# pyg-team/pytorch_geometric

Hardware: NVIDIA H100
Metric: edges/sec (GCNConv fwd+bwd) (higher is better)
Workload: dtype f32

## Files before the change

include/b200mp.h:

```cpp
#ifndef B200MP_H_
#define B200MP_H_

#include <stdint.h>

#ifdef __cplusplus
extern "C" {
#endif

#define B200MP_VERSION "0.1.0"

enum { B200MP_F32 = 0, B200MP_BF16 = 1 };
enum { B200MP_I32 = 0, B200MP_I64 = 1 };
enum { B200MP_SUM = 0, B200MP_MEAN = 1, B200MP_MIN = 2, B200MP_MAX = 3, B200MP_MUL = 4 };
enum {
    B200MP_OK = 0,
    B200MP_ERR_INVALID_ARG = -1,
    B200MP_ERR_UNSUPPORTED = -2,
    B200MP_ERR_CUDA = -3,
    B200MP_ERR_WORKSPACE = -4
};

const char* b200mp_version(void);
const char* b200mp_last_error(void);
int b200mp_device_info(int* sm_count, int* cc_major, int* cc_minor, int64_t* l2_bytes);
// ... 18 lines not shown
                         void* stream);
int64_t b200mp_self_loops_workspace_bytes(int64_t n_edges, int64_t n_nodes, int idx_dtype);
int b200mp_self_loops(const void* row, const void* col, const float* w_in, int64_t n_edges,
                      int64_t n_nodes, float fill_value, int mode, void* row_out, void* col_out,
                      float* w_out, int64_t* n_out_dev, void* workspace, int64_t workspace_bytes,
                      int idx_dtype, void* stream);
int b200mp_gcn_norm_csr(const void* rowptr, const void* src, const float* w, int64_t n_nodes,
                        int64_t n_edges, float* deg_inv_sqrt, float* w_out, int idx_dtype,
                        void* stream);

int b200mp_csr_plan_count(const void* rowptr, int64_t n_rows, int64_t chunk, int64_t* counts_dev,
                          int idx_dtype, void* stream);
int64_t b200mp_csr_plan_workspace_bytes(int64_t n_rows, int64_t n_long_rows, int idx_dtype);
int b200mp_csr_plan_fill(const void* rowptr, int64_t n_rows, int64_t chunk, int64_t n_long_rows,
                         int64_t* long_rows, int64_t* chunk_ptr, void* workspace,
                         int64_t workspace_bytes, int idx_dtype, void* stream);

int b200mp_spmm_csr(const void* rowptr, const void* col, const float* val, const void* x,
                    void* out, int64_t n_rows, int64_t n_cols, int64_t feat, int reduce,
                    const int64_t* long_rows, const int64_t* chunk_ptr, int64_t n_long_rows,
                    int64_t n_chunks, int64_t chunk, float* partials, const float* bias,
                    const void* x_halo, int64_t n_local_cols, int flags, const void* peer_ptrs,
                    int64_t peer_rows, const void* relu_mask, int idx_dtype, int val_dtype, void* stream);

int b200mp_segment_csr(const void* ptr, const void* src, void* out, int64_t n_rows, int64_t n_src,
                       int64_t feat, int reduce, const int64_t* long_rows, const int64_t* chunk_ptr,
                       int64_t n_long_rows, int64_t n_chunks, int64_t chunk, float* partials,
                       int idx_dtype, int val_dtype, void* stream);

int b200mp_minmax_ties(const void* rowptr, const void* col, const float* val, const void* x,
                       const void* out, float* ties, int64_t n_rows, int64_t feat,
                       int count_self_zero, int idx_dtype, int val_dtype, void* stream);
int b200mp_minmax_backward(const void* rowptr_t, const void* col_t, const float* val_t,
                           const void* x, const void* out, const void* grad_out, const float* ties,
                           void* grad_x, int64_t n_src, int64_t feat, int idx_dtype,
                           int val_dtype, void* stream);

int b200mp_sddmm_csr(const void* rowptr, const void* col, const void* a, const void* b, float* dot,
                     int64_t n_rows, int64_t feat, int idx_dtype, int val_dtype, void* stream);

int b200mp_edge_relu_csr(const void* rowptr, const void* col, const void* perm, const void* x,
                         const void* edge_rows, void* out, void* mask, int64_t n_rows, int64_t n_cols,
                         int64_t n_edges, int64_t feat, int reduce, const int64_t* long_rows,
                         const int64_t* chunk_ptr, int64_t n_long_rows, int64_t n_chunks, int64_t chunk,
                         float* partials, int idx_dtype, int val_dtype, void* stream);
int b200mp_edge_relu_backward_x(const void* rowptr_t, const void* col_t, const void* t2csr,
// ... 264 lines not shown
```

pytorch_geometric_b200/_lib.py:

```python
from __future__ import annotations

import ctypes
import os
import re

from . import _build

_I64 = ctypes.c_int64
_INT = ctypes.c_int
_P = ctypes.c_void_p
_F = ctypes.c_float
_U64 = ctypes.c_uint64

_SIGS = {
    "b200mp_version": (ctypes.c_char_p, []),
    "b200mp_last_error": (ctypes.c_char_p, []),
    "b200mp_device_info": (_INT, [_P, _P, _P, _P]),
    "b200mp_set_option": (_INT, [ctypes.c_char_p, _INT]),
    "b200mp_degree": (_INT, [_P, _I64, _I64, _P, _INT, _P]),
    "b200mp_index2ptr": (_INT, [_P, _I64, _I64, _P, _INT, _P]),
    "b200mp_ptr2index": (_INT, [_P, _I64, _I64, _P, _INT, _P]),
    "b200mp_index_stats": (_INT, [_P, _I64, _P, _INT, _P]),
    "b200mp_sort_workspace_bytes": (_I64, [_I64, _I64, _INT]),
    "b200mp_sort_by_key": (_INT, [_P, _I64, _I64, _P, _P, _P, _P, _I64, _INT, _P]),
    "b200mp_permute": (_INT, [_P, _P, _P, _I64, _INT, _INT, _P]),
    "b200mp_convert_index": (_INT, [_P, _INT, _P, _INT, _I64, _P]),
    "b200mp_self_loops_workspace_bytes": (_I64, [_I64, _I64, _INT]),
    "b200mp_self_loops": (_INT, [_P, _P, _P, _I64, _I64, _F, _INT, _P, _P, _P, _P, _P, _I64, _INT, _P]),
    "b200mp_gcn_norm_csr": (_INT, [_P, _P, _P, _I64, _I64, _P, _P, _INT, _P]),
    "b200mp_csr_plan_count": (_INT, [_P, _I64, _I64, _P, _INT, _P]),
    "b200mp_csr_plan_workspace_bytes": (_I64, [_I64, _I64, _INT]),
    "b200mp_csr_plan_fill": (_INT, [_P, _I64, _I64, _I64, _P, _P, _P, _I64, _INT, _P]),
    "b200mp_spmm_csr": (_INT, [_P, _P, _P, _P, _P, _I64, _I64, _I64, _INT, _P, _P, _I64, _I64, _I64, _P,
                               _P, _P, _I64, _INT, _P, _I64, _P, _INT, _INT, _P]),
    "b200mp_segment_csr": (_INT, [_P, _P, _P, _I64, _I64, _I64, _INT, _P, _P, _I64, _I64, _I64, _P, _INT, _INT, _P]),
    "b200mp_minmax_ties": (_INT, [_P, _P, _P, _P, _P, _P, _I64, _I64, _INT, _INT, _INT, _P]),
    "b200mp_minmax_backward": (_INT, [_P, _P, _P, _P, _P, _P, _P, _P, _I64, _I64, _INT, _INT, _P]),
    "b200mp_sddmm_csr": (_INT, [_P, _P, _P, _P, _P, _I64, _I64, _INT, _INT, _P]),
    "b200mp_edge_relu_csr": (_INT, [_P] * 7 + [_I64] * 4 + [_INT, _P, _P, _I64, _I64, _I64, _P, _INT, _INT, _P]),
    "b200mp_edge_relu_backward_x": (_INT, [_P] * 7 + [_I64, _I64, _P, _P, _I64, _I64, _I64, _P, _INT, _INT, _P]),
    "b200mp_edge_relu_backward_edge": (_INT, [_P] * 5 + [_I64, _I64, _INT, _P, _P, _I64, _I64, _I64, _INT, _INT, _P]),
    "b200mp_gated_csr": (_INT, [_P] * 6 + [_I64] * 5 + [_INT, _P, _P, _I64, _I64, _I64, _P, _INT, _INT, _P]),
    "b200mp_gated_backward_dst": (_INT, [_P] * 7 + [_I64] * 5 + [_INT, _P, _P, _I64, _I64, _I64, _P, _INT, _INT, _P]),
    "b200mp_gated_backward_src": (_INT, [_P] * 9 + [_I64] * 5 + [_P, _P, _I64, _I64, _I64, _P, _INT, _INT, _P]),
    "b200mp_cg_csr": (_INT, [_P] * 7 + [_I64] * 6 + [_INT, _P, _P, _I64, _I64, _I64, _P, _INT, _INT, _P]),
    "b200mp_cg_backward_dst": (_INT, [_P] * 9 + [_I64] * 6 + [_INT, _P, _P, _I64, _I64, _I64, _P, _INT, _INT, _P]),
    "b200mp_cg_backward_src": (_INT, [_P] * 9 + [_I64] * 6 + [_P, _P, _I64, _I64, _I64, _P, _INT, _INT, _P]),
    "b200mp_softmax_aggr_csr": (_INT, [_P] * 8 + [_I64] * 4 + [_INT, _F, _INT, _P, _P, _I64, _I64, _I64, _P, _INT, _INT,
                                                                _P]),
    "b200mp_softmax_aggr_workspace": (_I64, [_I64, _I64, _I64]),
    "b200mp_softmax_aggr_backward_dst": (_INT, [_P] * 12 + [_I64] * 4 + [_INT, _F, _INT, _INT, _P, _P, _I64, _I64, _I64,
                                                                           _INT, _INT, _P]),
    "b200mp_softmax_aggr_backward_src": (_INT, [_P] * 10 + [_I64] * 4 + [_INT, _F, _INT, _INT, _P, _P, _I64, _I64, _I64,
                                                                           _P, _INT, _INT, _P]),
    "b200mp_power_mean_csr": (_INT, [_P] * 8 + [_I64] * 4 + [_INT, _F, _INT, _F, _F, _P, _P, _I64, _I64, _I64, _P,
                                                              _INT, _INT, _P]),
    "b200mp_power_mean_workspace": (_I64, [_I64, _I64, _I64, _I64]),
# ... 100 lines not shown
```

pytorch_geometric_b200/csrc/csr_reduce.cuh:

```cuda
#pragma once

#include "common.cuh"

namespace b200mp {

int get_option_spmm_tune();

struct LongRowPlan {
    const int64_t* long_rows;
    const int64_t* chunk_ptr;
    int64_t n_long;
    int64_t n_chunks;
    int64_t chunk;
    float* partials;
    const void* x2;
    int64_t split;
    int accumulate;
    const unsigned long long* peers;
    int64_t peer_rows;
    const void* relu_mask;
};

inline int make_plan(LongRowPlan& plan, const int64_t* long_rows, const int64_t* chunk_ptr, int64_t n_long_rows,
                     int64_t n_chunks, int64_t chunk, float* partials, bool needs_partials) {
// ... 31 lines not shown
        is_chunk = true;
        return true;
    }
    row = item - plan.n_chunks;
    if (row >= n_rows) return false;
    begin = static_cast<int64_t>(__ldg(rowptr + row));
    end = static_cast<int64_t>(__ldg(rowptr + row + 1));
    is_chunk = false;
    if (plan.n_long > 0 && end - begin > plan.chunk) return false;
    return true;
}

template <int RED>
__device__ __forceinline__ float finalize(float acc, int64_t deg, bool is_mean, bool inf_to_zero) {
    if (RED == B200MP_SUM) {
        if (is_mean) acc = __fdiv_rn(acc, static_cast<float>(deg < 1 ? 1 : deg));
    } else if (RED == B200MP_MIN || RED == B200MP_MAX) {
        if (deg == 0) acc = 0.0f;
        if (inf_to_zero && isinf(acc)) acc = 0.0f;
    }
    return acc;
}

template <typename T, typename I, int G, int VPL, int RED, bool GATHER, int UNR_OVR = 0, int BLOCK = 256,
          int MINB = 1>
__global__ void __launch_bounds__(BLOCK, MINB)
csr_reduce_kernel(const I* __restrict__ rowptr, const I* __restrict__ col,
                  const float* __restrict__ val, const T* __restrict__ x, T* __restrict__ out,
                  int64_t n_rows, int n_vec, bool is_mean, bool inf_to_zero, LongRowPlan plan,
                  const float* __restrict__ bias) {
    constexpr int EPV = ElemTraits<T>::kPerVec;
    constexpr int UNR = UNR_OVR ? UNR_OVR : (VPL == 1 ? 8 : (VPL == 2 ? 4 : 2));
    const int lig = threadIdx.x & (G - 1);
    const int64_t item = (static_cast<int64_t>(blockIdx.x) * blockDim.x + threadIdx.x) / G;
    int64_t row, begin, end;
    bool is_chunk;
    const bool active = decode_item(item, rowptr, n_rows, plan, row, begin, end, is_chunk);
    if (G < 32 && !active) return;
    if (G == 32 && !active) return;
    const size_t row_bytes = static_cast<size_t>(n_vec) * 16;
    const char* xb = reinterpret_cast<const char*>(x);
    const char* xb2 = plan.x2 ? reinterpret_cast<const char*>(plan.x2) - static_cast<size_t>(plan.split) * row_bytes : xb;
    const int64_t split = plan.x2 ? plan.split : INT64_MAX;

    for (int vbase = 0; vbase < n_vec; vbase += G * VPL) {
        float acc[VPL][EPV];
#pragma unroll
        for (int k = 0; k < VPL; ++k)
#pragma unroll
            for (int i = 0; i < EPV; ++i) acc[k][i] = red_identity<RED>();
        bool vvalid[VPL];
#pragma unroll
        for (int k = 0; k < VPL; ++k) vvalid[k] = (vbase + lig + k * G) < n_vec;
        const size_t voff = static_cast<size_t>(vbase + lig) * 16;

        if (G == 32) {
            for (int64_t e0 = begin; e0 < end; e0 += 32) {
                const int n = static_cast<int>(end - e0 < 32 ? end - e0 : 32);
                int64_t c_l = 0;
                float w_l = 1.0f;
                if (lig < n) {
                    c_l = GATHER ? static_cast<int64_t>(ldg_idx(col + e0 + lig)) : (e0 + lig);
                    if (val) w_l = __ldg(val + e0 + lig);
                    c_l = static_cast<int64_t>(reinterpret_cast<uintptr_t>(row_base(plan, xb, xb2, split, row_bytes, c_l)));
                }
                for (int j = 0; j < n; j += UNR) {
                    Vec16 buf[UNR][VPL];
                    float w[UNR];
#pragma unroll
                    for (int u = 0; u < UNR; ++u) {
                        const int64_t c = __shfl_sync(0xffffffffu, c_l, (j + u) & 31);
                        w[u] = __shfl_sync(0xffffffffu, w_l, (j + u) & 31);
                        if (j + u < n) {
                            const char* p = reinterpret_cast<const char*>(static_cast<uintptr_t>(c)) + voff;
#pragma unroll
                            for (int k = 0; k < VPL; ++k)
                                if (vvalid[k]) buf[u][k] = ldg_row16(p + static_cast<size_t>(k) * G * 16);
                        }
                    }
#pragma unroll
                    for (int u = 0; u < UNR; ++u) {
                        if (j + u < n) {
#pragma unroll
                            for (int k = 0; k < VPL; ++k) {
                                if (vvalid[k]) {
                                    float f[EPV];
                                    ElemTraits<T>::unpack(buf[u][k], f);
#pragma unroll
                                    for (int i = 0; i < EPV; ++i) {
                                        const float m = val ? __fmul_rn(w[u], f[i]) : f[i];
                                        acc[k][i] = red_combine<RED>(acc[k][i], m);
                                    }
                                }
                            }
                        }
                    }
                }
            }
        } else {
            for (int64_t e = begin; e < end; e += UNR) {
                Vec16 buf[UNR][VPL];
                float w[UNR];
#pragma unroll
                for (int u = 0; u < UNR; ++u) {
                    w[u] = 1.0f;
                    if (e + u < end) {
                        const int64_t c = GATHER ? static_cast<int64_t>(ldg_idx(col + e + u)) : (e + u);
                        if (val) w[u] = __ldg(val + e + u);
                        if (vvalid[0]) buf[u][0] = ldg_row16(row_base(plan, xb, xb2, split, row_bytes, c) + voff);
                    }
                }
#pragma unroll
                for (int u = 0; u < UNR; ++u) {
                    if (e + u < end && vvalid[0]) {
                        float f[EPV];
                        ElemTraits<T>::unpack(buf[u][0], f);
#pragma unroll
                        for (int i = 0; i < EPV; ++i) {
                            const float m = val ? __fmul_rn(w[u], f[i]) : f[i];
                            acc[0][i] = red_combine<RED>(acc[0][i], m);
                        }
                    }
                }
            }
        }

        if (is_chunk) {
            float* pbase = plan.partials + static_cast<size_t>(item) * n_vec * EPV;
#pragma unroll
            for (int k = 0; k < VPL; ++k)
                if (vvalid[k]) store_partial<EPV>(pbase + static_cast<size_t>(vbase + lig + k * G) * EPV, acc[k]);
        } else {
            const int64_t deg = end - begin;
            char* ob = reinterpret_cast<char*>(out) + static_cast<size_t>(row) * row_bytes;
#pragma unroll
            for (int k = 0; k < VPL; ++k) {
                if (!vvalid[k]) continue;
                float f[EPV];
#pragma unroll
                for (int i = 0; i < EPV; ++i) f[i] = finalize<RED>(acc[k][i], deg, is_mean, inf_to_zero);
                if (bias) {
                    const float* bp = bias + static_cast<size_t>(vbase + lig + k * G) * EPV;
#pragma unroll
                    for (int i = 0; i < EPV; ++i) f[i] = __fadd_rn(f[i], __ldg(bp + i));
                }
                if (plan.accumulate) {
                    if (deg == 0 && !plan.relu_mask) continue;
                    float o[EPV];
                    ElemTraits<T>::unpack(*reinterpret_cast<const Vec16*>(ob + static_cast<size_t>(vbase + lig + k * G) * 16), o);
#pragma unroll
                    for (int i = 0; i < EPV; ++i) f[i] = deg == 0 ? o[i] : __fadd_rn(o[i], f[i]);
                    if (plan.relu_mask) {
                        float mk[EPV];
                        ElemTraits<T>::unpack(ldg_stream16(static_cast<const char*>(plan.relu_mask) + static_cast<size_t>(row) * row_bytes +
                                                           static_cast<size_t>(vbase + lig + k * G) * 16), mk);
#pragma unroll
                        for (int i = 0; i < EPV; ++i) f[i] = mk[i] > 0.0f ? f[i] : 0.0f;
                    }
                }
                stg_stream16(ob + static_cast<size_t>(vbase + lig + k * G) * 16, ElemTraits<T>::pack(f));
            }
        }
    }
}

template <typename T, typename I, int RED>
__global__ void __launch_bounds__(256)
csr_combine_kernel(const I* __restrict__ rowptr, T* __restrict__ out, int64_t feat, bool is_mean,
                   bool inf_to_zero, LongRowPlan plan, const float* __restrict__ bias) {
    const int64_t j = blockIdx.x;
    if (j >= plan.n_long) return;
    const int64_t row = plan.long_rows[j];
    const int64_t c0 = plan.chunk_ptr[j], c1 = plan.chunk_ptr[j + 1];
    const int64_t deg = static_cast<int64_t>(rowptr[row + 1]) - static_cast<int64_t>(rowptr[row]);
    for (int64_t f = threadIdx.x; f < feat; f += blockDim.x) {
        float acc = red_identity<RED>();
        for (int64_t c = c0; c < c1; ++c) acc = red_combine<RED>(acc, plan.partials[c * feat + f]);
        acc = finalize<RED>(acc, deg, is_mean, inf_to_zero);
        if (bias) acc = __fadd_rn(acc, bias[f]);
        if (plan.accumulate) acc = __fadd_rn(ElemTraits<T>::to_float(out[row * feat + f]), acc);
        if (plan.relu_mask && !(ElemTraits<T>::to_float(static_cast<const T*>(plan.relu_mask)[row * feat + f]) > 0.0f)) acc = 0.0f;
        out[row * feat + f] = ElemTraits<T>::from_float(acc);
    }
}

// ... 24 lines not shown
                                                       : x[c * feat + f]);
                }
            }
#pragma unroll
            for (int u = 0; u < 4; ++u)
                if (e + u < end) acc = red_combine<RED>(acc, val ? __fmul_rn(w[u], v[u]) : v[u]);
        }
        if (is_chunk)
            plan.partials[item * feat + f] = acc;
        else {
            acc = finalize<RED>(acc, end - begin, is_mean, inf_to_zero);
            if (bias) acc = __fadd_rn(acc, bias[f]);
            if (plan.accumulate) {
                if (end == begin && !plan.relu_mask) continue;
                const float o = ElemTraits<T>::to_float(out[row * feat + f]);
                acc = end == begin ? o : __fadd_rn(o, acc);
                if (plan.relu_mask && !(ElemTraits<T>::to_float(static_cast<const T*>(plan.relu_mask)[row * feat + f]) > 0.0f)) acc = 0.0f;
            }
            out[row * feat + f] = ElemTraits<T>::from_float(acc);
        }
    }
}

template <typename T, typename I, int RED, bool GATHER, int G, int VPL>
inline void launch_vec(const I* rowptr, const I* col, const float* val, const T* x, T* out,
                       int64_t n_rows, int n_vec, bool is_mean, bool inf_to_zero,
                       const LongRowPlan& plan, const float* bias, cudaStream_t stream) {
    const int64_t items = plan.n_chunks + n_rows;
    if (items == 0) return;
#define B200MP_LAUNCH_TUNED(UNR_, BLOCK_, MINB_)                                                           \
    csr_reduce_kernel<T, I, G, VPL, RED, GATHER, UNR_, BLOCK_, MINB_>                                      \
        <<<static_cast<unsigned>(ceil_div(items, BLOCK_ / G)), BLOCK_, 0, stream>>>(                       \
            rowptr, col, val, x, out, n_rows, n_vec, is_mean, inf_to_zero, plan, bias)
    if (G == 32 && VPL == 2 && RED == B200MP_SUM && GATHER) {
        switch (get_option_spmm_tune()) {
            case 1: B200MP_LAUNCH_TUNED(4, 256, 1); return;
            case 2: B200MP_LAUNCH_TUNED(4, 256, 4); return;
            case 3: B200MP_LAUNCH_TUNED(1, 256, 8); return;
            default: break;
        }
    }
    if (sizeof(T) == 4) B200MP_LAUNCH_TUNED(unroll_for_vpl<VPL>(), 128, 12);
    else B200MP_LAUNCH_TUNED(unroll_for_vpl<VPL>(), 128, 8);
#undef B200MP_LAUNCH_TUNED
}

template <typename T, typename I, int RED, bool GATHER>
int csr_reduce_dispatch(const I* rowptr, const I* col, const float* val, const T* x, T* out,
                        int64_t n_rows, int64_t feat, bool is_mean, bool inf_to_zero,
                        LongRowPlan plan, const float* bias, cudaStream_t stream) {
    if (n_rows == 0 || feat == 0) return B200MP_OK;
    const size_t row_bytes = static_cast<size_t>(feat) * sizeof(T);
    const bool vec_ok = (row_bytes % 16 == 0) && aligned16(x) && aligned16(out) && aligned16(plan.x2) &&
                        aligned16(plan.relu_mask) && (plan.n_chunks == 0 || aligned16(plan.partials));
    if (vec_ok) {
        const int n_vec = static_cast<int>(row_bytes / 16);
        lane_group_shape<4>(n_vec, [&](auto G, auto VPL) {
            launch_vec<T, I, RED, GATHER, G(), VPL()>(rowptr, col, val, x, out, n_rows, n_vec, is_mean, inf_to_zero,
                                                      plan, bias, stream);
        });
    } else {
        int g = 1;
        while (g < 32 && g < feat) g <<= 1;
        const int64_t items = plan.n_chunks + n_rows;
        const int64_t blocks = ceil_div(items, 256 / g);
        csr_reduce_scalar_kernel<T, I, RED, GATHER><<<static_cast<unsigned>(blocks), 256, 0, stream>>>(
            rowptr, col, val, x, out, n_rows, feat, g, is_mean, inf_to_zero, plan, bias);
    }
    B200MP_LAUNCH_CHECK();
    if (plan.n_long > 0) {
        csr_combine_kernel<T, I, RED><<<static_cast<unsigned>(plan.n_long), 256, 0, stream>>>(
            rowptr, out, feat, is_mean, inf_to_zero, plan, bias);
        B200MP_LAUNCH_CHECK();
    }
    return B200MP_OK;
}

template <typename T, typename I, bool GATHER>
int csr_reduce_by_op(const I* rowptr, const I* col, const float* val, const T* x, T* out,
                     int64_t n_rows, int64_t feat, int reduce, bool inf_to_zero, LongRowPlan plan,
                     const float* bias, cudaStream_t stream) {
    switch (reduce) {
        case B200MP_SUM:
            return csr_reduce_dispatch<T, I, B200MP_SUM, GATHER>(rowptr, col, val, x, out, n_rows, feat, false, false, plan, bias, stream);
        case B200MP_MEAN:
            return csr_reduce_dispatch<T, I, B200MP_SUM, GATHER>(rowptr, col, val, x, out, n_rows, feat, true, false, plan, bias, stream);
        case B200MP_MIN:
            return csr_reduce_dispatch<T, I, B200MP_MIN, GATHER>(rowptr, col, val, x, out, n_rows, feat, false, inf_to_zero, plan, bias, stream);
        case B200MP_MAX:
            return csr_reduce_dispatch<T, I, B200MP_MAX, GATHER>(rowptr, col, val, x, out, n_rows, feat, false, inf_to_zero, plan, bias, stream);
        default:
            set_error("csr_reduce: unsupported reduce %d", reduce);
            return B200MP_ERR_UNSUPPORTED;
    }
}

}
```

pytorch_geometric_b200/csrc/spmm.cu:

```cuda
#include "csr_dispatch.cuh"

namespace b200mp {

template <typename T, typename I>
__global__ void __launch_bounds__(256)
minmax_ties_kernel(const I* __restrict__ rowptr, const I* __restrict__ col,
                   const float* __restrict__ val, const T* __restrict__ x, const T* __restrict__ out,
                   float* __restrict__ ties, int64_t n_rows, int64_t feat, int g, bool count_self_zero) {
    const int lig = threadIdx.x & (g - 1);
    const int64_t row = (static_cast<int64_t>(blockIdx.x) * blockDim.x + threadIdx.x) / g;
    if (row >= n_rows) return;
    const int64_t begin = rowptr[row], end = rowptr[row + 1];
    for (int64_t f = lig; f < feat; f += g) {
        const float o = ElemTraits<T>::to_float(out[row * feat + f]);
        float cnt = (count_self_zero && o == 0.0f) ? 1.0f : 0.0f;
        for (int64_t e = begin; e < end; e += 4) {
            float v[4];
#pragma unroll
            for (int u = 0; u < 4; ++u) {
                v[u] = 0.f;
                if (e + u < end) {
                    const int64_t c = col[e + u];
                    const float xv = ElemTraits<T>::to_float(x[c * feat + f]);
                    v[u] = ElemTraits<T>::to_float(ElemTraits<T>::from_float(val ? __fmul_rn(__ldg(val + e + u), xv) : xv));
// ... 90 lines not shown
    if (int rc = make_plan(plan, long_rows, chunk_ptr, n_long_rows, n_chunks, chunk, partials, true)) return rc;
    if (n_rows == 0 || feat == 0) return B200MP_OK;
    B200MP_CHECK_ARG(rowptr && out);
    B200MP_CHECK_ARG(x || n_cols == 0 || peer_ptrs);
    B200MP_CHECK_ARG(!peer_ptrs || (peer_rows > 0 && !x_halo && (feat * (val_dtype == B200MP_BF16 ? 2 : 4)) % 16 == 0));
    B200MP_CHECK_ARG(!peer_ptrs || (aligned16(x) && aligned16(out) && aligned16(relu_mask) &&
                                    (n_long_rows == 0 || aligned16(partials))));
    B200MP_CHECK_ARG(!x_halo || (n_local_cols >= 0 && n_local_cols <= n_cols));
    plan.x2 = x_halo;
    plan.split = x_halo ? n_local_cols : 0;
    plan.accumulate = flags & 1;
    plan.peers = static_cast<const unsigned long long*>(peer_ptrs);
    plan.peer_rows = peer_ptrs ? peer_rows : 0;
    plan.relu_mask = relu_mask;
    return dispatch_val_idx(val_dtype, idx_dtype, "spmm_csr", [&](auto tv, auto ti) {
        using T = decltype(tv);
        using I = decltype(ti);
        return csr_reduce_auto<T, I, true>(static_cast<const I*>(rowptr), static_cast<const I*>(col), val,
                                            static_cast<const T*>(x), static_cast<T*>(out), n_rows, feat, reduce,
                                            false, plan, bias, static_cast<cudaStream_t>(stream));
    });
}

extern "C" int b200mp_minmax_ties(const void* rowptr, const void* col, const float* val, const void* x,
                                  const void* out, float* ties, int64_t n_rows, int64_t feat,
                                  int count_self_zero, int idx_dtype, int val_dtype, void* stream) {
    B200MP_CHECK_ARG(n_rows >= 0 && feat >= 0);
    if (n_rows == 0 || feat == 0) return B200MP_OK;
    B200MP_CHECK_ARG(rowptr && out && ties);
    return dispatch_val_idx(val_dtype, idx_dtype, "minmax_ties", [&](auto tv, auto ti) {
        using T = decltype(tv);
        using I = decltype(ti);
        const int g = group_width(feat);
        minmax_ties_kernel<T, I><<<static_cast<unsigned>(ceil_div(n_rows, 256 / g)), 256, 0,
                                   static_cast<cudaStream_t>(stream)>>>(
            static_cast<const I*>(rowptr), static_cast<const I*>(col), val, static_cast<const T*>(x),
            static_cast<const T*>(out), ties, n_rows, feat, g, count_self_zero != 0);
        B200MP_LAUNCH_CHECK();
        return B200MP_OK;
    });
}

extern "C" int b200mp_minmax_backward(const void* rowptr_t, const void* col_t, const float* val_t,
                                      const void* x, const void* out, const void* grad_out,
                                      const float* ties, void* grad_x, int64_t n_src, int64_t feat,
                                      int idx_dtype, int val_dtype, void* stream) {
// ... 34 lines not shown
```

pytorch_geometric_b200/graph.py:

```python
from __future__ import annotations

from typing import Optional

import torch
from torch import Tensor

from . import ops

DEFAULT_CHUNK = 512
_INT32_MAX = 2**31 - 1


class CSRGraph:
    def __init__(self, src: Tensor, dst: Tensor, num_src: int, num_dst: int,
                 edge_weight: Optional[Tensor] = None, chunk: int = DEFAULT_CHUNK,
                 idx_dtype: Optional[torch.dtype] = None):
        if not src.is_cuda:
            raise RuntimeError("CSRGraph lives on a CUDA device (no CPU fallback)")
        E = src.numel()
        if idx_dtype is None:
            idx_dtype = torch.int32 if max(num_src, num_dst, E) < _INT32_MAX else torch.int64
        self.idx_dtype = idx_dtype
        self.num_src, self.num_dst, self.num_edges = int(num_src), int(num_dst), int(E)
        self.chunk = int(chunk)
        self.device = src.device
        self._src = ops.convert_index(src.contiguous(), idx_dtype)
        self._dst = ops.convert_index(dst.contiguous(), idx_dtype)
        _, self.perm, self.rowptr = ops.sort_by_key(self._dst, self.num_dst, want_sorted=False)
        self.col = ops.permute(self._src, self.perm)
        self.val = None if edge_weight is None else ops.permute(edge_weight.detach().float().contiguous(), self.perm)
        self.plan = ops.LongRowPlan(self.rowptr, self.chunk)
        self._t_built = False
        self.perm_t = self.rowptr_t = self.col_t = self.val_t = self.plan_t = None
        self._mean_val_t = None
        self._inv_perm = None
        self._inv_perm_t = None
# ... 207 lines not shown
```

pytorch_geometric_b200/nn/conv.py:

```python
from __future__ import annotations

import math
from typing import Optional, Union

import torch
import torch.nn.functional as F
from torch import Tensor

from .. import dense
from .. import functional as Fn
from .. import ops
from .. import utils as U
from ..graph import CSRGraph, cached_graph

Adj = Union[Tensor, CSRGraph]


def glorot_(w: Tensor) -> Tensor:
    a = math.sqrt(6.0 / (w.size(-2) + w.size(-1)))
    with torch.no_grad():
        return w.uniform_(-a, a)


class _Lin(torch.nn.Module):
# ... 6 lines not shown

    def forward(self, x: Tensor) -> Tensor:
        return dense.linear(x, self.weight, self.bias)


def _w(mod):
    return None if mod is None else mod.weight


class _BiasAggregate(torch.autograd.Function):

    @staticmethod
    def forward(ctx, x: Tensor, bias: Tensor, graph: CSRGraph):
        ctx.graph = graph
        return ops.spmm_csr(graph.rowptr, graph.col, graph.val, x, graph.num_dst, "sum", graph.plan, bias=bias)

    @staticmethod
    def backward(ctx, grad_out: Tensor):
        graph = ctx.graph
        grad_out = grad_out.contiguous()
        gx = gb = None
        if ctx.needs_input_grad[0]:
            graph.build_transpose()
            gx = ops.spmm_csr(graph.rowptr_t, graph.col_t, graph.val_t, grad_out, graph.num_src, "sum", graph.plan_t)
        if ctx.needs_input_grad[1]:
            gb = ops.column_sum(grad_out)
        return gx, gb, None


def gcn_conv(x: Tensor, graph: CSRGraph, weight: Tensor, bias: Optional[Tensor]) -> Tensor:
    xw = dense.linear(x, weight)
    if bias is not None:
        return _BiasAggregate.apply(xw, bias, graph)
    return Fn.aggregate(graph, xw, "sum")


class _SageFused(torch.autograd.Function):

    @staticmethod
    def forward(ctx, x: Tensor, w_l: Tensor, b_l: Optional[Tensor], w_r: Tensor, graph: CSRGraph, aggr: str, relu: bool,
                input_is_relu: bool, grad_masked_by_consumer: bool):
        x = x.contiguous()
        agg = ops.spmm_csr(graph.rowptr, graph.col, graph.val, x, graph.num_dst, aggr, graph.plan)
        w_hi, w_lo = dense.split_tf32(torch.cat([w_l.detach(), w_r.detach()], dim=1))
        y, _ = dense.gemm_pair(agg, x, w_hi, w_lo, 0, w_l.size(0), bias=None if b_l is None else b_l.detach(), relu=relu)
        ctx.graph, ctx.aggr, ctx.relu, ctx.has_bias = graph, aggr, relu, b_l is not None
        ctx.input_is_relu, ctx.premasked = input_is_relu, grad_masked_by_consumer
        ctx.save_for_backward(x, agg, w_hi, w_lo, y if (relu and not grad_masked_by_consumer) else None)
# ... 1034 lines not shown
```

pytorch_geometric_b200/ops.py:

```python
from __future__ import annotations

import ctypes
from typing import Optional, Tuple

import torch
from torch import Tensor

from ._lib import check, lib

F32, BF16 = 0, 1
I32, I64 = 0, 1
REDUCE = {"sum": 0, "add": 0, "mean": 1, "min": 2, "amin": 2, "max": 3, "amax": 3, "mul": 4}


class _Launches:
    count = 0


LAUNCHES = _Launches()


class _Profile:

    def __init__(self):
# ... 233 lines not shown
        args = (_p(plan.long_rows), _p(plan.chunk_ptr), plan.n_long, plan.n_chunks, plan.chunk, _p(part))
    else:
        args = (None, None, 0, 0, 0, None)
    if bias is not None:
        _cuda(bias)
        if bias.dtype != torch.float32 or not bias.is_contiguous():
            bias = bias.detach().float().contiguous()
        if bias.numel() != F:
            raise ValueError("bias must have one entry per feature")
    if relu_mask is not None:
        _cuda(relu_mask)
        if not accumulate or relu_mask.dtype != x.dtype or tuple(relu_mask.shape) != (n_rows, F) or not relu_mask.is_contiguous():
            raise ValueError("relu_mask needs accumulate=True and a contiguous [n_rows, F] tensor of x's dtype")
    n_cols, n_local = x.size(0), 0
    if x_halo is not None:
        _cuda(x_halo)
        if x_halo.dtype != x.dtype or x_halo.dim() != 2 or x_halo.size(1) != F or not x_halo.is_contiguous():
            raise ValueError("x_halo must be a contiguous [n_halo, F] tensor of x's dtype")
        n_local, n_cols = x.size(0), x.size(0) + x_halo.size(0)
    _timed("spmm_csr", 2 if args[2] else 1, lib().b200mp_spmm_csr, _p(rowptr), _p(col), _p(val), _p(x), _p(out),
           n_rows, n_cols, F, REDUCE[reduce], *args, _p(bias), _p(x_halo), n_local, int(bool(accumulate)),
           peer_ptrs, int(peer_rows), _p(relu_mask), it, _vdt(x), _stream())
    return out


SEGMENT_PLAN_MIN_ROWS = 1 << 16
SEGMENT_CHUNK = 512


_PLAN_CACHE: "dict" = {}
_PLAN_CACHE_MAX = 32


def segment_plan(ptr: Tensor, n_src: int) -> Optional["LongRowPlan"]:
    if n_src < SEGMENT_PLAN_MIN_ROWS:
        return None
    import weakref
    key = id(ptr)
    hit = _PLAN_CACHE.get(key)
    if hit is not None and hit[0]() is ptr and hit[1] == ptr._version:
        return hit[2]
    plan = LongRowPlan(ptr, SEGMENT_CHUNK)
    plan = plan if plan.n_long else None
    if len(_PLAN_CACHE) >= _PLAN_CACHE_MAX:
        for k in [k for k, v in _PLAN_CACHE.items() if v[0]() is None] or list(_PLAN_CACHE)[:1]:
            _PLAN_CACHE.pop(k, None)
# ... 1015 lines not shown
```

pytorch_geometric_b200/utils.py:

```python
from __future__ import annotations

from typing import Optional, Tuple, Union

import torch
from torch import Tensor

from . import functional as Fn
from . import ops
from .graph import CSRGraph


def _move_dim0(src: Tensor, dim: int) -> Tuple[Tensor, bool]:
    if dim == 0:
        return src, False
    return src.movedim(dim, 0).contiguous(), True


def scatter(src: Tensor, index: Tensor, dim: int = 0, dim_size: Optional[int] = None, reduce: str = "sum",
            sorted: Optional[bool] = None) -> Tensor:
    if isinstance(index, Tensor) and index.dim() != 1:
        raise ValueError(f"The `index` argument must be one-dimensional (got {index.dim()} dimensions)")
    dim = src.dim() + dim if dim < 0 else dim
    if dim < 0 or dim >= src.dim():
        raise ValueError(f"The `dim` argument must lay between 0 and {src.dim() - 1} (got {dim})")
# ... 129 lines not shown


def gcn_norm(edge_index: Tensor, edge_weight: Optional[Tensor] = None, num_nodes: Optional[int] = None,
             improved: bool = False, add_self_loops: bool = True, flow: str = "source_to_target",
             dtype: Optional[torch.dtype] = None) -> Tuple[Tensor, Tensor]:
    g, ei = gcn_norm_graph(edge_index, edge_weight, num_nodes, improved, add_self_loops, flow, return_edge_index=True)
    return ei, g.from_csr_order(g.val)


def gcn_norm_graph(edge_index: Tensor, edge_weight: Optional[Tensor] = None, num_nodes: Optional[int] = None,
                   improved: bool = False, add_self_loops: bool = True, flow: str = "source_to_target",
                   return_edge_index: bool = False, chunk: Optional[int] = None):
    assert flow in ("source_to_target", "target_to_source")
    if edge_weight is not None and edge_weight.requires_grad:
        raise NotImplementedError("gcn_norm with edge_weight.requires_grad is not supported by the fused path")
    N = num_nodes if num_nodes is not None else ((ops.index_stats(edge_index.reshape(-1))[1] + 1)
                                                  if edge_index.numel() else 0)
    row, col, w = edge_index[0], edge_index[1], edge_weight
    if add_self_loops:
        row, col, w = ops.self_loops(row, col, w, N, 2.0 if improved else 1.0, 0)
    src, dst = (row, col) if flow == "source_to_target" else (col, row)
    kw = {} if chunk is None else {"chunk": chunk}
    g = CSRGraph(src, dst, N, N, None, **kw)
    w_csr = None if w is None else g.to_csr_order(w.float())
    _, w_norm = ops.gcn_norm_csr(g.rowptr, g.col, w_csr)
    g.val = w_norm
    if return_edge_index:
        return g, torch.stack([row, col])
    return g


def spmm(src: Union[CSRGraph, Tensor], other: Tensor, reduce: str = "sum") -> Tensor:
    reduce = "sum" if reduce == "add" else reduce
    if reduce not in ("sum", "mean", "min", "max"):
        raise ValueError(f"`reduce` argument '{reduce}' not supported")
    if isinstance(src, CSRGraph):
        return Fn.aggregate(src, other, reduce)
    if isinstance(src, Tensor) and src.layout == torch.sparse_csr:
        rowptr, col, val = src.crow_indices(), src.col_indices(), src.values()
        n_rows = src.size(0)
        if other.requires_grad or val.requires_grad:
            raise NotImplementedError("pass a CSRGraph for a differentiable spmm")
        return ops.spmm_csr(rowptr, col, val.float(), other, n_rows, reduce)
    raise ValueError("`src` must be a CSRGraph or a torch.sparse_csr tensor")
```

Measured before the change: 920.6 million.

## Fuse bias-gradient column sum into transposed SpMM via self-loop rows

In GCNConv backward, the bias gradient (column sum of grad_out) is computed inside the transposed SpMM kernel. Each source row's self-loop edge already loads grad_out[row], so the kernel adds that unweighted row into a per-block shared-memory slot, and a small reduction over the per-block partials finishes the sum. This removes a separate full pass over grad_out, at the cost of shared memory per lane group, a persistent-style grid sized from occupancy, and an extra partials reduction. It relies on the graph having exactly one self loop per row, which is flagged when gcn_norm adds self loops.

New measurement: 967.9 million (median of 6 runs). 1.05x the previous value.

```diff
diff --git a/include/b200mp.h b/include/b200mp.h
--- a/include/b200mp.h
+++ b/include/b200mp.h
@@ -64,6 +64,12 @@
                     int64_t n_chunks, int64_t chunk, float* partials, const float* bias,
                     const void* x_halo, int64_t n_local_cols, int flags, const void* peer_ptrs,
                     int64_t peer_rows, const void* relu_mask, int idx_dtype, int val_dtype, void* stream);
+
+int b200mp_spmm_csr_self_colsum(const void* rowptr_t, const void* col_t, const float* val_t, const void* x, void* out,
+                                float* colsum_out, int64_t n_rows, int64_t feat, const int64_t* long_rows_t,
+                                const int64_t* chunk_ptr_t, int64_t n_long_rows_t, int64_t n_chunks_t, int64_t chunk,
+                                float* partials_t, float* colsum_parts, int64_t n_parts, int idx_dtype, int val_dtype,
+                                void* stream);
 
 int b200mp_segment_csr(const void* ptr, const void* src, void* out, int64_t n_rows, int64_t n_src,
                        int64_t feat, int reduce, const int64_t* long_rows, const int64_t* chunk_ptr,
diff --git a/pytorch_geometric_b200/_lib.py b/pytorch_geometric_b200/_lib.py
--- a/pytorch_geometric_b200/_lib.py
+++ b/pytorch_geometric_b200/_lib.py
@@ -33,6 +33,8 @@
     "b200mp_csr_plan_fill": (_INT, [_P, _I64, _I64, _I64, _P, _P, _P, _I64, _INT, _P]),
     "b200mp_spmm_csr": (_INT, [_P, _P, _P, _P, _P, _I64, _I64, _I64, _INT, _P, _P, _I64, _I64, _I64, _P,
                                _P, _P, _I64, _INT, _P, _I64, _P, _INT, _INT, _P]),
+    "b200mp_spmm_csr_self_colsum": (_INT, [_P, _P, _P, _P, _P, _P, _I64, _I64, _P, _P, _I64, _I64, _I64, _P, _P, _I64,
+                                           _INT, _INT, _P]),
     "b200mp_segment_csr": (_INT, [_P, _P, _P, _I64, _I64, _I64, _INT, _P, _P, _I64, _I64, _I64, _P, _INT, _INT, _P]),
     "b200mp_minmax_ties": (_INT, [_P, _P, _P, _P, _P, _P, _I64, _I64, _INT, _INT, _INT, _P]),
     "b200mp_minmax_backward": (_INT, [_P, _P, _P, _P, _P, _P, _P, _P, _I64, _I64, _INT, _INT, _P]),
diff --git a/pytorch_geometric_b200/csrc/csr_reduce.cuh b/pytorch_geometric_b200/csrc/csr_reduce.cuh
--- a/pytorch_geometric_b200/csrc/csr_reduce.cuh
+++ b/pytorch_geometric_b200/csrc/csr_reduce.cuh
@@ -1,4 +1,6 @@
 #pragma once
+
+#include <algorithm>
 
 #include "common.cuh"
 
@@ -77,145 +79,194 @@
     return acc;
 }
 
+template <int EPV>
+__device__ __forceinline__ void add_to_slot(float* s, const float (&f)[EPV]) {
+#pragma unroll
+    for (int q = 0; q < EPV / 4; ++q) {
+        float4 t = reinterpret_cast<float4*>(s)[q];
+        t.x += f[4 * q];
+        t.y += f[4 * q + 1];
+        t.z += f[4 * q + 2];
+        t.w += f[4 * q + 3];
+        reinterpret_cast<float4*>(s)[q] = t;
+    }
+}
+
 template <typename T, typename I, int G, int VPL, int RED, bool GATHER, int UNR_OVR = 0, int BLOCK = 256,
-          int MINB = 1>
+          int MINB = 1, bool SELF_COLSUM = false>
 __global__ void __launch_bounds__(BLOCK, MINB)
 csr_reduce_kernel(const I* __restrict__ rowptr, const I* __restrict__ col,
                   const float* __restrict__ val, const T* __restrict__ x, T* __restrict__ out,
                   int64_t n_rows, int n_vec, bool is_mean, bool inf_to_zero, LongRowPlan plan,
-                  const float* __restrict__ bias) {
+                  const float* __restrict__ bias, float* __restrict__ colsum_parts) {
+    static_assert(!SELF_COLSUM || (RED == B200MP_SUM && GATHER), "the self-loop column sum rides a weighted-sum gather");
     constexpr int EPV = ElemTraits<T>::kPerVec;
     constexpr int UNR = UNR_OVR ? UNR_OVR : (VPL == 1 ? 8 : (VPL == 2 ? 4 : 2));
+    constexpr int GROUPS = BLOCK / G;
+    extern __shared__ float4 csr_colsum_smem[];
     const int lig = threadIdx.x & (G - 1);
-    const int64_t item = (static_cast<int64_t>(blockIdx.x) * blockDim.x + threadIdx.x) / G;
-    int64_t row, begin, end;
-    bool is_chunk;
-    const bool active = decode_item(item, rowptr, n_rows, plan, row, begin, end, is_chunk);
-    if (G < 32 && !active) return;
-    if (G == 32 && !active) return;
+    const int feat = n_vec * EPV;
+    float* const slot = reinterpret_cast<float*>(csr_colsum_smem) + static_cast<size_t>(threadIdx.x / G) * feat;
     const size_t row_bytes = static_cast<size_t>(n_vec) * 16;
     const char* xb = reinterpret_cast<const char*>(x);
     const char* xb2 = plan.x2 ? reinterpret_cast<const char*>(plan.x2) - static_cast<size_t>(plan.split) * row_bytes : xb;
     const int64_t split = plan.x2 ? plan.split : INT64_MAX;
-
-    for (int vbase = 0; vbase < n_vec; vbase += G * VPL) {
-        float acc[VPL][EPV];
-#pragma unroll
-        for (int k = 0; k < VPL; ++k)
-#pragma unroll
-            for (int i = 0; i < EPV; ++i) acc[k][i] = red_identity<RED>();
-        bool vvalid[VPL];
-#pragma unroll
-        for (int k = 0; k < VPL; ++k) vvalid[k] = (vbase + lig + k * G) < n_vec;
-        const size_t voff = static_cast<size_t>(vbase + lig) * 16;
-
-        if (G == 32) {
-            for (int64_t e0 = begin; e0 < end; e0 += 32) {
-                const int n = static_cast<int>(end - e0 < 32 ? end - e0 : 32);
-                int64_t c_l = 0;
-                float w_l = 1.0f;
-                if (lig < n) {
-                    c_l = GATHER ? static_cast<int64_t>(ldg_idx(col + e0 + lig)) : (e0 + lig);
-                    if (val) w_l = __ldg(val + e0 + lig);
-                    c_l = static_cast<int64_t>(reinterpret_cast<uintptr_t>(row_base(plan, xb, xb2, split, row_bytes, c_l)));
-                }
-                for (int j = 0; j < n; j += UNR) {
-                    Vec16 buf[UNR][VPL];
-                    float w[UNR];
-#pragma unroll
-                    for (int u = 0; u < UNR; ++u) {
-                        const int64_t c = __shfl_sync(0xffffffffu, c_l, (j + u) & 31);
-                        w[u] = __shfl_sync(0xffffffffu, w_l, (j + u) & 31);
-                        if (j + u < n) {
-                            const char* p = reinterpret_cast<const char*>(static_cast<uintptr_t>(c)) + voff;
-#pragma unroll
-                            for (int k = 0; k < VPL; ++k)
-                                if (vvalid[k]) buf[u][k] = ldg_row16(p + static_cast<size_t>(k) * G * 16);
+    const bool weighted = SELF_COLSUM || val;
+    auto src_row = [&](int64_t c) {
+        return SELF_COLSUM ? xb + static_cast<size_t>(c) * row_bytes : row_base(plan, xb, xb2, split, row_bytes, c);
+    };
+
+    auto reduce_item = [&](const int64_t item) {
+        int64_t row, begin, end;
+        bool is_chunk;
+        const bool active = decode_item(item, rowptr, n_rows, plan, row, begin, end, is_chunk);
+        if (G < 32 && !active) return;
+        if (G == 32 && !active) return;
+
+        for (int vbase = 0; vbase < n_vec; vbase += G * VPL) {
+            float acc[VPL][EPV];
+#pragma unroll
+            for (int k = 0; k < VPL; ++k)
+#pragma unroll
+                for (int i = 0; i < EPV; ++i) acc[k][i] = red_identity<RED>();
+            bool vvalid[VPL];
+#pragma unroll
+            for (int k = 0; k < VPL; ++k) vvalid[k] = (vbase + lig + k * G) < n_vec;
+            const size_t voff = static_cast<size_t>(vbase + lig) * 16;
+
+            if (G == 32) {
+                for (int64_t e0 = begin; e0 < end; e0 += 32) {
+                    const int n = static_cast<int>(end - e0 < 32 ? end - e0 : 32);
+                    int64_t c_l = 0;
+                    float w_l = 1.0f;
+                    bool self_l = false;
+                    if (lig < n) {
+                        c_l = GATHER ? static_cast<int64_t>(ldg_idx(col + e0 + lig)) : (e0 + lig);
+                        if (weighted) w_l = __ldg(val + e0 + lig);
+                        if (SELF_COLSUM) self_l = c_l == row;
+                        c_l = static_cast<int64_t>(reinterpret_cast<uintptr_t>(src_row(c_l)));
+                    }
+                    const unsigned self_bits = SELF_COLSUM ? __ballot_sync(0xffffffffu, self_l) : 0u;
+                    for (int j = 0; j < n; j += UNR) {
+                        Vec16 buf[UNR][VPL];
+                        float w[UNR];
+#pragma unroll
+                        for (int u = 0; u < UNR; ++u) {
+                            const int64_t c = __shfl_sync(0xffffffffu, c_l, (j + u) & 31);
+                            w[u] = __shfl_sync(0xffffffffu, w_l, (j + u) & 31);
+                            if (j + u < n) {
+                                const char* p = reinterpret_cast<const char*>(static_cast<uintptr_t>(c)) + voff;
+#pragma unroll
+                                for (int k = 0; k < VPL; ++k)
+                                    if (vvalid[k]) buf[u][k] = ldg_row16(p + static_cast<size_t>(k) * G * 16);
+                            }
                         }
-                    }
-#pragma unroll
-                    for (int u = 0; u < UNR; ++u) {
-                        if (j + u < n) {
-#pragma unroll
-                            for (int k = 0; k < VPL; ++k) {
-                                if (vvalid[k]) {
-                                    float f[EPV];
-                                    ElemTraits<T>::unpack(buf[u][k], f);
-#pragma unroll
-                                    for (int i = 0; i < EPV; ++i) {
-                                        const float m = val ? __fmul_rn(w[u], f[i]) : f[i];
-                                        acc[k][i] = red_combine<RED>(acc[k][i], m);
+#pragma unroll
+                        for (int u = 0; u < UNR; ++u) {
+                            if (j + u < n) {
+#pragma unroll
+                                for (int k = 0; k < VPL; ++k) {
+                                    if (vvalid[k]) {
+                                        float f[EPV];
+                                        ElemTraits<T>::unpack(buf[u][k], f);
+#pragma unroll
+                                        for (int i = 0; i < EPV; ++i) {
+                                            const float m = weighted ? __fmul_rn(w[u], f[i]) : f[i];
+                                            acc[k][i] = red_combine<RED>(acc[k][i], m);
+                                        }
+                                        if (SELF_COLSUM && ((self_bits >> (j + u)) & 1u))
+                                            add_to_slot<EPV>(slot + static_cast<size_t>(vbase + lig + k * G) * EPV, f);
                                     }
                                 }
                             }
                         }
                     }
                 }
-            }
-        } else {
-            for (int64_t e = begin; e < end; e += UNR) {
-                Vec16 buf[UNR][VPL];
-                float w[UNR];
-#pragma unroll
-                for (int u = 0; u < UNR; ++u) {
-                    w[u] = 1.0f;
-                    if (e + u < end) {
-                        const int64_t c = GATHER ? static_cast<int64_t>(ldg_idx(col + e + u)) : (e + u);
-                        if (val) w[u] = __ldg(val + e + u);
-                        if (vvalid[0]) buf[u][0] = ldg_row16(row_base(plan, xb, xb2, split, row_bytes, c) + voff);
-                    }
-                }
-#pragma unroll
-                for (int u = 0; u < UNR; ++u) {
-                    if (e + u < end && vvalid[0]) {
-                        float f[EPV];
-                        ElemTraits<T>::unpack(buf[u][0], f);
-#pragma unroll
-                        for (int i = 0; i < EPV; ++i) {
-                            const float m = val ? __fmul_rn(w[u], f[i]) : f[i];
-                            acc[0][i] = red_combine<RED>(acc[0][i], m);
+            } else {
+                for (int64_t e = begin; e < end; e += UNR) {
+                    Vec16 buf[UNR][VPL];
+                    float w[UNR];
+                    unsigned self_bits = 0;
+#pragma unroll
+                    for (int u = 0; u < UNR; ++u) {
+                        w[u] = 1.0f;
+                        if (e + u < end) {
+                            const int64_t c = GATHER ? static_cast<int64_t>(ldg_idx(col + e + u)) : (e + u);
+                            if (weighted) w[u] = __ldg(val + e + u);
+                            if (SELF_COLSUM && c == row) self_bits |= 1u << u;
+                            if (vvalid[0]) buf[u][0] = ldg_row16(src_row(c) + voff);
+                        }
+                    }
+#pragma unroll
+                    for (int u = 0; u < UNR; ++u) {
+                        if (e + u < end && vvalid[0]) {
+                            float f[EPV];
+                            ElemTraits<T>::unpack(buf[u][0], f);
+#pragma unroll
+                            for (int i = 0; i < EPV; ++i) {
+                                const float m = weighted ? __fmul_rn(w[u], f[i]) : f[i];
+                                acc[0][i] = red_combine<RED>(acc[0][i], m);
+                            }
+                            if (SELF_COLSUM && ((self_bits >> u) & 1u))
+                                add_to_slot<EPV>(slot + static_cast<size_t>(vbase + lig) * EPV, f);
                         }
                     }
                 }
             }
-        }
-
-        if (is_chunk) {
-            float* pbase = plan.partials + static_cast<size_t>(item) * n_vec * EPV;
-#pragma unroll
-            for (int k = 0; k < VPL; ++k)
-                if (vvalid[k]) store_partial<EPV>(pbase + static_cast<size_t>(vbase + lig + k * G) * EPV, acc[k]);
-        } else {
-            const int64_t deg = end - begin;
-            char* ob = reinterpret_cast<char*>(out) + static_cast<size_t>(row) * row_bytes;
-#pragma unroll
-            for (int k = 0; k < VPL; ++k) {
-                if (!vvalid[k]) continue;
-                float f[EPV];
-#pragma unroll
-                for (int i = 0; i < EPV; ++i) f[i] = finalize<RED>(acc[k][i], deg, is_mean, inf_to_zero);
-                if (bias) {
-                    const float* bp = bias + static_cast<size_t>(vbase + lig + k * G) * EPV;
-#pragma unroll
-                    for (int i = 0; i < EPV; ++i) f[i] = __fadd_rn(f[i], __ldg(bp + i));
+
+            if (is_chunk) {
+                float* pbase = plan.partials + static_cast<size_t>(item) * n_vec * EPV;
+#pragma unroll
+                for (int k = 0; k < VPL; ++k)
+                    if (vvalid[k]) store_partial<EPV>(pbase + static_cast<size_t>(vbase + lig + k * G) * EPV, acc[k]);
+            } else {
+                const int64_t deg = end - begin;
+                char* ob = reinterpret_cast<char*>(out) + static_cast<size_t>(row) * row_bytes;
+#pragma unroll
+                for (int k = 0; k < VPL; ++k) {
+                    if (!vvalid[k]) continue;
+                    float f[EPV];
+#pragma unroll
+                    for (int i = 0; i < EPV; ++i) f[i] = finalize<RED>(acc[k][i], deg, !SELF_COLSUM && is_mean, inf_to_zero);
+                    if (!SELF_COLSUM && bias) {
+                        const float* bp = bias + static_cast<size_t>(vbase + lig + k * G) * EPV;
+#pragma unroll
+                        for (int i = 0; i < EPV; ++i) f[i] = __fadd_rn(f[i], __ldg(bp + i));
+                    }
+                    if (!SELF_COLSUM && plan.accumulate) {
+                        if (deg == 0 && !plan.relu_mask) continue;
+                        float o[EPV];
+                        ElemTraits<T>::unpack(*reinterpret_cast<const Vec16*>(ob + static_cast<size_t>(vbase + lig + k * G) * 16), o);
+#pragma unroll
+                        for (int i = 0; i < EPV; ++i) f[i] = deg == 0 ? o[i] : __fadd_rn(o[i], f[i]);
+                        if (plan.relu_mask) {
+                            float mk[EPV];
+                            ElemTraits<T>::unpack(ldg_stream16(static_cast<const char*>(plan.relu_mask) + static_cast<size_t>(row) * row_bytes +
+                                                               static_cast<size_t>(vbase + lig + k * G) * 16), mk);
+#pragma unroll
+                            for (int i = 0; i < EPV; ++i) f[i] = mk[i] > 0.0f ? f[i] : 0.0f;
+                        }
+                    }
+                    stg_stream16(ob + static_cast<size_t>(vbase + lig + k * G) * 16, ElemTraits<T>::pack(f));
                 }
-                if (plan.accumulate) {
-                    if (deg == 0 && !plan.relu_mask) continue;
-                    float o[EPV];
-                    ElemTraits<T>::unpack(*reinterpret_cast<const Vec16*>(ob + static_cast<size_t>(vbase + lig + k * G) * 16), o);
-#pragma unroll
-                    for (int i = 0; i < EPV; ++i) f[i] = deg == 0 ? o[i] : __fadd_rn(o[i], f[i]);
-                    if (plan.relu_mask) {
-                        float mk[EPV];
-                        ElemTraits<T>::unpack(ldg_stream16(static_cast<const char*>(plan.relu_mask) + static_cast<size_t>(row) * row_bytes +
-                                                           static_cast<size_t>(vbase + lig + k * G) * 16), mk);
-#pragma unroll
-                        for (int i = 0; i < EPV; ++i) f[i] = mk[i] > 0.0f ? f[i] : 0.0f;
-                    }
-                }
-                stg_stream16(ob + static_cast<size_t>(vbase + lig + k * G) * 16, ElemTraits<T>::pack(f));
             }
         }
+    };
+
+    const int64_t first = (static_cast<int64_t>(blockIdx.x) * blockDim.x + threadIdx.x) / G;
+    if constexpr (SELF_COLSUM) {
+        for (int i = threadIdx.x; i < GROUPS * feat; i += BLOCK) reinterpret_cast<float*>(csr_colsum_smem)[i] = 0.0f;
+        __syncthreads();
+        const int64_t n_items = plan.n_chunks + n_rows;
+        for (int64_t item = first; item < n_items; item += static_cast<int64_t>(gridDim.x) * GROUPS) reduce_item(item);
+        __syncthreads();
+        for (int f = threadIdx.x; f < feat; f += BLOCK) {
+            float s = 0.0f;
+            for (int q = 0; q < GROUPS; ++q) s += reinterpret_cast<const float*>(csr_colsum_smem)[q * feat + f];
+            colsum_parts[static_cast<size_t>(blockIdx.x) * feat + f] = s;
+        }
+    } else {
+        reduce_item(first);
     }
 }
 
@@ -286,6 +337,10 @@
     }
 }
 
+constexpr int kCsrBlock = 128;
+template <typename T>
+constexpr int csr_min_blocks() { return sizeof(T) == 4 ? 12 : 8; }
+
 template <typename T, typename I, int RED, bool GATHER, int G, int VPL>
 inline void launch_vec(const I* rowptr, const I* col, const float* val, const T* x, T* out,
                        int64_t n_rows, int n_vec, bool is_mean, bool inf_to_zero,
@@ -295,7 +350,7 @@
 #define B200MP_LAUNCH_TUNED(UNR_, BLOCK_, MINB_)                                                           \
     csr_reduce_kernel<T, I, G, VPL, RED, GATHER, UNR_, BLOCK_, MINB_>                                      \
         <<<static_cast<unsigned>(ceil_div(items, BLOCK_ / G)), BLOCK_, 0, stream>>>(                       \
-            rowptr, col, val, x, out, n_rows, n_vec, is_mean, inf_to_zero, plan, bias)
+            rowptr, col, val, x, out, n_rows, n_vec, is_mean, inf_to_zero, plan, bias, nullptr)
     if (G == 32 && VPL == 2 && RED == B200MP_SUM && GATHER) {
         switch (get_option_spmm_tune()) {
             case 1: B200MP_LAUNCH_TUNED(4, 256, 1); return;
@@ -304,8 +359,7 @@
             default: break;
         }
     }
-    if (sizeof(T) == 4) B200MP_LAUNCH_TUNED(unroll_for_vpl<VPL>(), 128, 12);
-    else B200MP_LAUNCH_TUNED(unroll_for_vpl<VPL>(), 128, 8);
+    B200MP_LAUNCH_TUNED(unroll_for_vpl<VPL>(), kCsrBlock, csr_min_blocks<T>());
 #undef B200MP_LAUNCH_TUNED
 }
 
@@ -340,6 +394,50 @@
     return B200MP_OK;
 }
 
+constexpr int kSelfColsumMinBlocks = 8;
+
+template <typename T, typename I>
+int csr_sum_self_colsum(const I* rowptr, const I* col, const float* val, const T* x, T* out, int64_t n_rows,
+                        int64_t feat, const LongRowPlan& plan, float* colsum_parts, int64_t max_parts, int64_t& parts,
+                        cudaStream_t stream) {
+    parts = 0;
+    const size_t row_bytes = static_cast<size_t>(feat) * sizeof(T);
+    if (row_bytes % 16 != 0 || !aligned16(x) || !aligned16(out) || (plan.n_chunks != 0 && !aligned16(plan.partials)))
+        return B200MP_OK;
+    const int n_vec = static_cast<int>(row_bytes / 16);
+    const int64_t items = plan.n_chunks + n_rows;
+    cudaError_t err = cudaSuccess;
+    lane_group_shape<4>(n_vec, [&](auto G, auto VPL) {
+        auto kernel = csr_reduce_kernel<T, I, G(), VPL(), B200MP_SUM, true, unroll_for_vpl<VPL()>(), kCsrBlock,
+                                        kSelfColsumMinBlocks, true>;
+        const size_t smem = static_cast<size_t>(kCsrBlock / G()) * feat * sizeof(float);
+        if (smem > 48 * 1024) return;
+        int dev = 0, smem_sm = 0;
+        if ((err = cudaGetDevice(&dev)) != cudaSuccess ||
+            (err = cudaDeviceGetAttribute(&smem_sm, cudaDevAttrMaxSharedMemoryPerMultiprocessor, dev)) != cudaSuccess)
+            return;
+        const int64_t need = static_cast<int64_t>(kSelfColsumMinBlocks) * (smem + 1024) * 100;
+        const int pct = static_cast<int>(std::min<int64_t>(100, ceil_div(need, smem_sm)));
+        if ((err = cudaFuncSetAttribute(kernel, cudaFuncAttributePreferredSharedMemoryCarveout, pct)) != cudaSuccess) return;
+        int per_sm = 0;
+        err = cudaOccupancyMaxActiveBlocksPerMultiprocessor(&per_sm, kernel, kCsrBlock, smem);
+        if (err != cudaSuccess) return;
+        parts = std::min(std::min(static_cast<int64_t>(per_sm) * num_sms(), ceil_div(items, kCsrBlock / G())),
+                         max_parts);
+        if (parts == 0) return;
+        kernel<<<static_cast<unsigned>(parts), kCsrBlock, smem, stream>>>(rowptr, col, val, x, out, n_rows, n_vec, false,
+                                                                           false, plan, nullptr, colsum_parts);
+    });
+    B200MP_CUDA(err);
+    B200MP_LAUNCH_CHECK();
+    if (parts > 0 && plan.n_long > 0) {
+        csr_combine_kernel<T, I, B200MP_SUM><<<static_cast<unsigned>(plan.n_long), 256, 0, stream>>>(
+            rowptr, out, feat, false, false, plan, nullptr);
+        B200MP_LAUNCH_CHECK();
+    }
+    return B200MP_OK;
+}
+
 template <typename T, typename I, bool GATHER>
 int csr_reduce_by_op(const I* rowptr, const I* col, const float* val, const T* x, T* out,
                      int64_t n_rows, int64_t feat, int reduce, bool inf_to_zero, LongRowPlan plan,
diff --git a/pytorch_geometric_b200/csrc/spmm.cu b/pytorch_geometric_b200/csrc/spmm.cu
--- a/pytorch_geometric_b200/csrc/spmm.cu
+++ b/pytorch_geometric_b200/csrc/spmm.cu
@@ -136,6 +136,39 @@
     });
 }
 
+extern "C" int b200mp_spmm_csr_self_colsum(const void* rowptr_t, const void* col_t, const float* val_t, const void* x,
+                                           void* out, float* colsum_out, int64_t n_rows, int64_t feat,
+                                           const int64_t* long_rows_t, const int64_t* chunk_ptr_t, int64_t n_long_rows_t,
+                                           int64_t n_chunks_t, int64_t chunk, float* partials_t, float* colsum_parts,
+                                           int64_t n_parts, int idx_dtype, int val_dtype, void* stream) {
+    B200MP_CHECK_ARG(n_rows >= 0 && feat >= 0 && n_parts >= 1);
+    LongRowPlan plan;
+    if (int rc = make_plan(plan, long_rows_t, chunk_ptr_t, n_long_rows_t, n_chunks_t, chunk, partials_t, true)) return rc;
+    if (feat == 0) return B200MP_OK;
+    B200MP_CHECK_ARG(colsum_out && colsum_parts);
+    cudaStream_t s = static_cast<cudaStream_t>(stream);
+    if (n_rows == 0) return b200mp_column_sum(nullptr, colsum_out, colsum_parts, 1, 0, feat, val_dtype, stream);
+    B200MP_CHECK_ARG(rowptr_t && col_t && val_t && x && out);
+    return dispatch_val_idx(val_dtype, idx_dtype, "spmm_csr_self_colsum", [&](auto tv, auto ti) {
+        using T = decltype(tv);
+        using I = decltype(ti);
+        int64_t parts = 0;
+        if (int rc = csr_sum_self_colsum<T, I>(static_cast<const I*>(rowptr_t), static_cast<const I*>(col_t), val_t,
+                                               static_cast<const T*>(x), static_cast<T*>(out), n_rows, feat, plan,
+                                               colsum_parts, n_parts - ceil_div(n_parts, 64), parts, s))
+            return rc;
+        if (parts > 0)
+            return b200mp_column_sum(colsum_parts, colsum_out, colsum_parts + parts * feat, b200mp_column_sum_parts(parts),
+                                     parts, feat, B200MP_F32, stream);
+        if (int rc = csr_reduce_dispatch<T, I, B200MP_SUM, true>(static_cast<const I*>(rowptr_t), static_cast<const I*>(col_t),
+                                                                 val_t, static_cast<const T*>(x), static_cast<T*>(out),
+                                                                 n_rows, feat, false, false, plan, nullptr, s))
+            return rc;
+        return b200mp_column_sum(x, colsum_out, colsum_parts, std::min(n_parts, b200mp_column_sum_parts(n_rows)), n_rows,
+                                 feat, val_dtype, stream);
+    });
+}
+
 extern "C" int b200mp_minmax_ties(const void* rowptr, const void* col, const float* val, const void* x,
                                   const void* out, float* ties, int64_t n_rows, int64_t feat,
                                   int count_self_zero, int idx_dtype, int val_dtype, void* stream) {
diff --git a/pytorch_geometric_b200/graph.py b/pytorch_geometric_b200/graph.py
--- a/pytorch_geometric_b200/graph.py
+++ b/pytorch_geometric_b200/graph.py
@@ -12,6 +12,8 @@
 
 
 class CSRGraph:
+    one_self_loop_per_row = False
+
     def __init__(self, src: Tensor, dst: Tensor, num_src: int, num_dst: int,
                  edge_weight: Optional[Tensor] = None, chunk: int = DEFAULT_CHUNK,
                  idx_dtype: Optional[torch.dtype] = None):
diff --git a/pytorch_geometric_b200/nn/conv.py b/pytorch_geometric_b200/nn/conv.py
--- a/pytorch_geometric_b200/nn/conv.py
+++ b/pytorch_geometric_b200/nn/conv.py
@@ -52,8 +52,11 @@
         gx = gb = None
         if ctx.needs_input_grad[0]:
             graph.build_transpose()
-            gx = ops.spmm_csr(graph.rowptr_t, graph.col_t, graph.val_t, grad_out, graph.num_src, "sum", graph.plan_t)
-        if ctx.needs_input_grad[1]:
+            if ctx.needs_input_grad[1] and graph.one_self_loop_per_row and graph.val_t is not None:
+                gx, gb = ops.spmm_csr_self_colsum(graph.rowptr_t, graph.col_t, graph.val_t, grad_out, graph.plan_t)
+            else:
+                gx = ops.spmm_csr(graph.rowptr_t, graph.col_t, graph.val_t, grad_out, graph.num_src, "sum", graph.plan_t)
+        if ctx.needs_input_grad[1] and gb is None:
             gb = ops.column_sum(grad_out)
         return gx, gb, None
 
diff --git a/pytorch_geometric_b200/ops.py b/pytorch_geometric_b200/ops.py
--- a/pytorch_geometric_b200/ops.py
+++ b/pytorch_geometric_b200/ops.py
@@ -279,6 +279,28 @@
            n_rows, n_cols, F, REDUCE[reduce], *args, _p(bias), _p(x_halo), n_local, int(bool(accumulate)),
            peer_ptrs, int(peer_rows), _p(relu_mask), it, _vdt(x), _stream())
     return out
+
+
+def spmm_csr_self_colsum(rowptr: Tensor, col: Tensor, val: Tensor, x: Tensor,
+                         plan: Optional[LongRowPlan] = None) -> Tuple[Tensor, Tensor]:
+    _cuda(rowptr, col, val, x)
+    if x.dim() != 2 or x.size(0) != rowptr.numel() - 1:
+        raise ValueError("spmm_csr_self_colsum expects a square graph and an [N, F] feature matrix")
+    x = x.contiguous()
+    it = _same_idx(rowptr, col)
+    val = val.contiguous().float()
+    n, F = x.shape
+    out = torch.empty(n, F, dtype=x.dtype, device=x.device)
+    colsum = torch.empty(F, dtype=torch.float32, device=x.device)
+    parts = 16 * torch.cuda.get_device_properties(x.device).multi_processor_count
+    ws = torch.empty(parts * max(F, 1), dtype=torch.float32, device=x.device)
+    if plan is not None and plan.n_long:
+        args = (_p(plan.long_rows), _p(plan.chunk_ptr), plan.n_long, plan.n_chunks, plan.chunk, _p(plan.partials(F, x.device)))
+    else:
+        args = (None, None, 0, 0, 0, None)
+    _timed("spmm_csr", 3 if args[2] else 2, lib().b200mp_spmm_csr_self_colsum, _p(rowptr), _p(col), _p(val), _p(x),
+           _p(out), _p(colsum), n, F, *args, _p(ws), parts, it, _vdt(x), _stream())
+    return out, colsum
 
 
 SEGMENT_PLAN_MIN_ROWS = 1 << 16
diff --git a/pytorch_geometric_b200/utils.py b/pytorch_geometric_b200/utils.py
--- a/pytorch_geometric_b200/utils.py
+++ b/pytorch_geometric_b200/utils.py
@@ -175,6 +175,7 @@
     src, dst = (row, col) if flow == "source_to_target" else (col, row)
     kw = {} if chunk is None else {"chunk": chunk}
     g = CSRGraph(src, dst, N, N, None, **kw)
+    g.one_self_loop_per_row = add_self_loops
     w_csr = None if w is None else g.to_csr_order(w.float())
     _, w_norm = ops.gcn_norm_csr(g.rowptr, g.col, w_csr)
     g.val = w_norm
```
